# danieldugas/DeepMimic_mujoco

Hardware: AMD Instinct MI355X
Metric: env-steps/sec (whole node), 34-DoF humanoid, 4096 envs, at 1/2/4/8 MI355X (higher is better)
Workload: dtype f32

## Files before the change

### deepmimic_mujoco_amd/csrc/dm_kernels.hip

```cpp
#include "../../include/deepmimic_hip.h"
#include "dm_device.h"
#include "dm_rng.h"
#include "dm_topology.h"

#include <math.h>

#include <type_traits>

#define SYNC()                                              \
  do {                                                      \
    __builtin_amdgcn_fence(__ATOMIC_RELEASE, "wavefront");  \
    __builtin_amdgcn_wave_barrier();                        \
    __builtin_amdgcn_fence(__ATOMIC_ACQUIRE, "wavefront");  \
  } while (0)
#define DMK_ENVS_PER_BLOCK 1
#ifndef DMK_WAVES_PER_SIMD
#define DMK_WAVES_PER_SIMD 2
#endif
#ifdef DM_PROFILE
#define PROF_DECL do { if ((threadIdx.x & 63) == 0) { for (int _i = 0; _i < 16; _i++) g_S.prof[_i] = 0; for (int _i = 0; _i < 4; _i++) g_S.prof_stage[_i] = 0; g_S.prof_t = g_S.prof_t0 = __builtin_amdgcn_s_memtime(); } } while (0)
#define PROF_STAGE(i) do { if ((threadIdx.x & 63) == 0 && (i) < 4) g_S.prof_stage[i] = (unsigned)(__builtin_amdgcn_s_memtime() - g_S.prof_t0); } while (0)
#define PROF(i) do { if ((threadIdx.x & 63) == 0) { unsigned long long _t = __builtin_amdgcn_s_memtime(); g_S.prof[i] += (unsigned)(_t - g_S.prof_t); g_S.prof_t = _t; } } while (0)
#if DM_PROFILE == 2
#define PROF2(i) PROF(i)
// ... 28 lines not shown
namespace {

template <int I, int N>
struct StaticFor {
  template <class F>
  static __device__ __forceinline__ void run(F &&f) {
    if constexpr (I < N) {
      if (f(std::integral_constant<int, I>{})) StaticFor<I + 1, N>::run(f);
    }
  }
};

__device__ __forceinline__ float rl(float v, int lane) {
  return __int_as_float(__builtin_amdgcn_readlane(__float_as_int(v), lane));
}
template <unsigned long long MASK>
__device__ __forceinline__ float lane_sel(float a, float b) {
  float out;
  asm("v_cndmask_b32_e64 %0, %1, %2, %3" : "=v"(out) : "v"(b), "v"(a), "s"(MASK));
  return out;
}
template <unsigned long long MASK>
__device__ __forceinline__ int lane_sel_i(int a, int b) {
  int out;
  asm("v_cndmask_b32_e64 %0, %1, %2, %3" : "=v"(out) : "v"(b), "v"(a), "s"(MASK));
  return out;
}
template <int N>
__device__ __forceinline__ void sgpr_batch(float (&a)[topo::FS_SLOTS]) {
  static_assert(N >= 1 && N <= 8 && topo::FS_SLOTS == 8, "one asm statement per batch size");
  if constexpr (N == 1) asm("" : "+s"(a[0]));
  if constexpr (N == 2) asm("" : "+s"(a[0]), "+s"(a[1]));
  if constexpr (N == 3) asm("" : "+s"(a[0]), "+s"(a[1]), "+s"(a[2]));
  if constexpr (N == 4) asm("" : "+s"(a[0]), "+s"(a[1]), "+s"(a[2]), "+s"(a[3]));
  if constexpr (N == 5) asm("" : "+s"(a[0]), "+s"(a[1]), "+s"(a[2]), "+s"(a[3]), "+s"(a[4]));
  if constexpr (N == 6) asm("" : "+s"(a[0]), "+s"(a[1]), "+s"(a[2]), "+s"(a[3]), "+s"(a[4]), "+s"(a[5]));
  if constexpr (N == 7) asm("" : "+s"(a[0]), "+s"(a[1]), "+s"(a[2]), "+s"(a[3]), "+s"(a[4]), "+s"(a[5]), "+s"(a[6]));
  if constexpr (N == 8) asm("" : "+s"(a[0]), "+s"(a[1]), "+s"(a[2]), "+s"(a[3]), "+s"(a[4]), "+s"(a[5]), "+s"(a[6]), "+s"(a[7]));
}
__device__ __forceinline__ void factor_columns(float (&C)[DMK_NV]) {
  float d[topo::FS_SLOTS], m[topo::FS_SLOTS], rk[DMK_NV], Cs[DMK_NV];
  StaticFor<0, topo::FS_NOPS>::run([&](auto nc) {
    constexpr topo::FactorOp o = topo::FACTOR_SCHED[decltype(nc)::value];
    if constexpr (o.op == topo::FS_DIAG) d[o.slot] = rl(C[o.k], o.k);
    if constexpr (o.op == topo::FS_RCP) rk[o.k] = __builtin_amdgcn_rcpf(d[o.slot]);
    if constexpr (o.op == topo::FS_SCALE) Cs[o.k] = C[o.k] * rk[o.k];
    if constexpr (o.op == topo::FS_BCAST) m[o.slot] = rl(Cs[o.k], o.i);
    if constexpr (o.op == topo::FS_FMA) C[o.i] = fmaf(-m[o.slot], C[o.k], C[o.i]);
    if constexpr (o.op == topo::FS_FENCE) sgpr_batch<o.slot>(m);
    if constexpr (o.op == topo::FS_DFENCE) sgpr_batch<o.slot>(d);
    return true;
  });
}
__device__ __forceinline__ float solve_LT(float x, const float dv, const int negdep, const float *M) {
  StaticFor<0, DMK_NV - 1>::run([&](auto ic) {
    constexpr int i = DMK_NV - 1 - decltype(ic)::value;
    const float xi = rl(x * dv, i);
    const float l = lane_sel<topo::anc_mask(i)>(M[topo::MADR[i] + topo::NANC[i] + negdep], 0.f);
    x = fmaf(-l, xi, x);
    return true;
  });
  return x;
}
__device__ __forceinline__ float solve_L(float x, const float dv, const int mrow, const float *M) {
  StaticFor<0, DMK_NV - 1>::run([&](auto jc) {
    constexpr int j = decltype(jc)::value;
    const float xj = rl(x * dv, j);
    const float l = lane_sel<topo::desc_mask(j)>(M[mrow - topo::NANC[j]], 0.f);
    x = fmaf(-l, xj, x);
    return true;
  });
  return x;
}
template <int I, int K = 0>
__device__ __forceinline__ void load_factor_row(lds_cfloat_p Sp, float (&W)[DMK_MAXANC], float &dinv) {
  static_assert(alignof(EnvLds) >= 16 && offsetof(EnvLds, M) % 4 == 0 && offsetof(EnvLds, dinv) % 4 == 0, "EnvLds layout");
  constexpr int n = topo::NANC[I];
  constexpr int a = (int)(offsetof(EnvLds, M) / 4) + topo::MADR[I] + 1 + K;
  if constexpr (K >= n) {
    dinv = Sp[offsetof(EnvLds, dinv) / 4 + I];
  } else if constexpr (a % 4 == 0 && n - K >= 4) {
    const lds_f4v v = *reinterpret_cast<__attribute__((address_space(3))) const lds_f4v *>(Sp + a);
    W[K] = v.x; W[K + 1] = v.y; W[K + 2] = v.z; W[K + 3] = v.w;
    load_factor_row<I, K + 4>(Sp, W, dinv);
  } else if constexpr (a % 2 == 0 && n - K >= 2) {
    const lds_f2v v = *reinterpret_cast<__attribute__((address_space(3))) const lds_f2v *>(Sp + a);
    W[K] = v.x; W[K + 1] = v.y;
    load_factor_row<I, K + 2>(Sp, W, dinv);
  } else {
    W[K] = Sp[a];
    load_factor_row<I, K + 1>(Sp, W, dinv);
  }
}
template <int CTRL>
__device__ __forceinline__ float dpp_mov(float v) {
  return __int_as_float(__builtin_amdgcn_update_dpp(0, __float_as_int(v), CTRL, 0xF, 0xF, true));
}
__device__ __forceinline__ float wave_sum(float v) {
  v += dpp_mov<0xB1>(v);
  v += dpp_mov<0x4E>(v);
  v += dpp_mov<0x141>(v);
  v += dpp_mov<0x140>(v);
  return (rl(v, 0) + rl(v, 16)) + (rl(v, 32) + rl(v, 48));
}
__device__ __forceinline__ unsigned long long lanemask_lt(int lane) {
  return (lane == 0) ? 0ull : (~0ull >> (64 - lane));
}
__device__ __forceinline__ int prefix_count(bool flag, int lane, int *total) {
  unsigned long long m = __ballot(flag);
  *total = __popcll(m);
  return __popcll(m & lanemask_lt(lane));
}

__device__ __forceinline__ void cross3(float *r, const float *a, const float *b) {
  float x = a[1] * b[2] - a[2] * b[1], y = a[2] * b[0] - a[0] * b[2], z = a[0] * b[1] - a[1] * b[0];
  r[0] = x; r[1] = y; r[2] = z;
}
__device__ __forceinline__ float dot3(const float *a, const float *b) {
  return a[0] * b[0] + a[1] * b[1] + a[2] * b[2];
}
__device__ __forceinline__ void quat_mul(float *r, const float *a, const float *b) {
  float w = a[0] * b[0] - a[1] * b[1] - a[2] * b[2] - a[3] * b[3];
  float x = a[0] * b[1] + a[1] * b[0] + a[2] * b[3] - a[3] * b[2];
  float y = a[0] * b[2] - a[1] * b[3] + a[2] * b[0] + a[3] * b[1];
  float z = a[0] * b[3] + a[1] * b[2] - a[2] * b[1] + a[3] * b[0];
// ... 1867 lines not shown
```

### deepmimic_mujoco_amd/csrc/dm_topology.h

```cpp
#pragma once
namespace topo {
constexpr int NV = 34;
constexpr int NM = 310;
constexpr int PARENT[NV] = {-1, 0, 1, 2, 3, 4, 5, 6, 7, 8, 9, 10, 8, 12, 13, 14, 8, 16, 17, 18, 5, 20, 21, 22, 23, 24, 25, 5, 27, 28, 29, 30, 31, 32};
constexpr int NANC[NV] = {0, 1, 2, 3, 4, 5, 6, 7, 8, 9, 10, 11, 9, 10, 11, 12, 9, 10, 11, 12, 6, 7, 8, 9, 10, 11, 12, 6, 7, 8, 9, 10, 11, 12};
constexpr int MADR[NV] = {0, 1, 3, 6, 10, 15, 21, 28, 36, 45, 55, 66, 78, 88, 99, 111, 124, 134, 145, 157, 170, 177, 185, 194, 204, 215, 227, 240, 247, 255, 264, 274, 285, 297};
constexpr bool is_anc(int j, int i) {
  for (int a = PARENT[i]; a >= 0; a = PARENT[a]) if (a == j) return true;
  return false;
}
constexpr int midx(int i, int j) { return MADR[i] + NANC[i] - NANC[j]; }
constexpr int NB = 14;
constexpr int BPARENT[NB] = {0, 0, 1, 2, 2, 4, 2, 6, 1, 8, 9, 1, 11, 12};
constexpr unsigned long long body_ancself_mask(int c) {
  unsigned long long m = 0;
  for (int b = c; b >= 1; b = BPARENT[b]) m |= 1ull << b;
  return m;
}
constexpr unsigned long long desc_mask(int j) {
  unsigned long long m = 0;
  for (int i = 0; i < NV; i++) if (is_anc(j, i)) m |= 1ull << i;
  return m;
}
constexpr unsigned long long anc_mask(int i) {
// ... 75 lines not shown
  {FS_FMA, 19, 3, 7}, {FS_BCAST, 19, 2, 0}, {FS_BCAST, 19, 1, 1}, {FS_BCAST, 19, 0, 2}, {FS_BCAST, 18, 8, 3}, {FS_BCAST, 18, 7, 4},
  {FS_BCAST, 18, 6, 5}, {FS_BCAST, 18, 5, 6}, {FS_BCAST, 18, 4, 7}, {FS_FENCE, 0, 0, 8}, {FS_FMA, 19, 2, 0}, {FS_FMA, 19, 1, 1},
  {FS_FMA, 19, 0, 2}, {FS_FMA, 18, 8, 3}, {FS_FMA, 18, 7, 4}, {FS_FMA, 18, 6, 5}, {FS_FMA, 18, 5, 6}, {FS_FMA, 18, 4, 7},
  {FS_BCAST, 18, 3, 0}, {FS_BCAST, 18, 2, 1}, {FS_BCAST, 18, 1, 2}, {FS_BCAST, 18, 0, 3}, {FS_BCAST, 17, 8, 4}, {FS_BCAST, 17, 7, 5},
  {FS_BCAST, 17, 6, 6}, {FS_BCAST, 17, 5, 7}, {FS_FENCE, 0, 0, 8}, {FS_FMA, 18, 3, 0}, {FS_FMA, 18, 2, 1}, {FS_FMA, 18, 1, 2},
  {FS_FMA, 18, 0, 3}, {FS_FMA, 17, 8, 4}, {FS_FMA, 17, 7, 5}, {FS_FMA, 17, 6, 6}, {FS_FMA, 17, 5, 7}, {FS_BCAST, 17, 4, 0},
  {FS_BCAST, 17, 3, 1}, {FS_BCAST, 17, 2, 2}, {FS_BCAST, 17, 1, 3}, {FS_BCAST, 17, 0, 4}, {FS_BCAST, 16, 8, 5}, {FS_BCAST, 16, 7, 6},
  {FS_BCAST, 16, 6, 7}, {FS_FENCE, 0, 0, 8}, {FS_FMA, 17, 4, 0}, {FS_FMA, 17, 3, 1}, {FS_FMA, 17, 2, 2}, {FS_FMA, 17, 1, 3},
  {FS_FMA, 17, 0, 4}, {FS_FMA, 16, 8, 5}, {FS_FMA, 16, 7, 6}, {FS_FMA, 16, 6, 7}, {FS_BCAST, 16, 5, 0}, {FS_BCAST, 16, 4, 1},
  {FS_BCAST, 16, 3, 2}, {FS_BCAST, 16, 2, 3}, {FS_BCAST, 16, 1, 4}, {FS_BCAST, 16, 0, 5}, {FS_BCAST, 15, 8, 6}, {FS_BCAST, 15, 7, 7},
  {FS_FENCE, 0, 0, 8}, {FS_FMA, 16, 5, 0}, {FS_FMA, 16, 4, 1}, {FS_FMA, 16, 3, 2}, {FS_FMA, 16, 2, 3}, {FS_FMA, 16, 1, 4},
  {FS_FMA, 16, 0, 5}, {FS_FMA, 15, 8, 6}, {FS_FMA, 15, 7, 7}, {FS_BCAST, 15, 6, 0}, {FS_BCAST, 15, 5, 1}, {FS_BCAST, 15, 4, 2},
  {FS_BCAST, 15, 3, 3}, {FS_BCAST, 15, 2, 4}, {FS_BCAST, 15, 1, 5}, {FS_BCAST, 15, 0, 6}, {FS_BCAST, 14, 8, 7}, {FS_FENCE, 0, 0, 8},
  {FS_FMA, 15, 6, 0}, {FS_FMA, 15, 5, 1}, {FS_FMA, 15, 4, 2}, {FS_FMA, 15, 3, 3}, {FS_FMA, 15, 2, 4}, {FS_FMA, 15, 1, 5},
  {FS_FMA, 15, 0, 6}, {FS_FMA, 14, 8, 7}, {FS_BCAST, 14, 7, 0}, {FS_BCAST, 14, 6, 1}, {FS_BCAST, 14, 5, 2}, {FS_BCAST, 14, 4, 3},
  {FS_BCAST, 14, 3, 4}, {FS_BCAST, 14, 2, 5}, {FS_BCAST, 14, 1, 6}, {FS_BCAST, 14, 0, 7}, {FS_FENCE, 0, 0, 8}, {FS_FMA, 14, 7, 0},
  {FS_FMA, 14, 6, 1}, {FS_FMA, 14, 5, 2}, {FS_FMA, 14, 4, 3}, {FS_FMA, 14, 3, 4}, {FS_FMA, 14, 2, 5}, {FS_FMA, 14, 1, 6},
  {FS_FMA, 14, 0, 7}, {FS_BCAST, 13, 8, 0}, {FS_BCAST, 13, 7, 1}, {FS_BCAST, 13, 6, 2}, {FS_BCAST, 13, 5, 3}, {FS_BCAST, 13, 4, 4},
  {FS_BCAST, 13, 3, 5}, {FS_BCAST, 13, 2, 6}, {FS_BCAST, 13, 1, 7}, {FS_FENCE, 0, 0, 8}, {FS_FMA, 13, 8, 0}, {FS_FMA, 13, 7, 1},
  {FS_FMA, 13, 6, 2}, {FS_FMA, 13, 5, 3}, {FS_FMA, 13, 4, 4}, {FS_FMA, 13, 3, 5}, {FS_FMA, 13, 2, 6}, {FS_FMA, 13, 1, 7},
  {FS_BCAST, 13, 0, 0}, {FS_BCAST, 12, 8, 1}, {FS_BCAST, 12, 7, 2}, {FS_BCAST, 12, 6, 3}, {FS_BCAST, 12, 5, 4}, {FS_BCAST, 12, 4, 5},
  {FS_BCAST, 12, 3, 6}, {FS_BCAST, 12, 2, 7}, {FS_FENCE, 0, 0, 8}, {FS_FMA, 13, 0, 0}, {FS_FMA, 12, 8, 1}, {FS_FMA, 12, 7, 2},
  {FS_FMA, 12, 6, 3}, {FS_FMA, 12, 5, 4}, {FS_FMA, 12, 4, 5}, {FS_FMA, 12, 3, 6}, {FS_FMA, 12, 2, 7}, {FS_BCAST, 12, 1, 0},
  {FS_BCAST, 12, 0, 1}, {FS_BCAST, 11, 8, 2}, {FS_BCAST, 11, 7, 3}, {FS_BCAST, 11, 6, 4}, {FS_BCAST, 11, 5, 5}, {FS_BCAST, 11, 4, 6},
  {FS_BCAST, 11, 3, 7}, {FS_FENCE, 0, 0, 8}, {FS_FMA, 12, 1, 0}, {FS_FMA, 12, 0, 1}, {FS_FMA, 11, 8, 2}, {FS_FMA, 11, 7, 3},
  {FS_FMA, 11, 6, 4}, {FS_FMA, 11, 5, 5}, {FS_FMA, 11, 4, 6}, {FS_FMA, 11, 3, 7}, {FS_BCAST, 11, 2, 0}, {FS_BCAST, 11, 1, 1},
  {FS_BCAST, 11, 0, 2}, {FS_BCAST, 10, 8, 3}, {FS_BCAST, 10, 7, 4}, {FS_BCAST, 10, 6, 5}, {FS_BCAST, 10, 5, 6}, {FS_BCAST, 10, 4, 7},
  {FS_FENCE, 0, 0, 8}, {FS_FMA, 11, 2, 0}, {FS_FMA, 11, 1, 1}, {FS_FMA, 11, 0, 2}, {FS_FMA, 10, 8, 3}, {FS_FMA, 10, 7, 4},
  {FS_FMA, 10, 6, 5}, {FS_FMA, 10, 5, 6}, {FS_FMA, 10, 4, 7}, {FS_BCAST, 10, 3, 0}, {FS_BCAST, 10, 2, 1}, {FS_BCAST, 10, 1, 2},
  {FS_BCAST, 10, 0, 3}, {FS_BCAST, 9, 8, 4}, {FS_BCAST, 9, 7, 5}, {FS_BCAST, 9, 6, 6}, {FS_BCAST, 9, 5, 7}, {FS_FENCE, 0, 0, 8},
  {FS_FMA, 10, 3, 0}, {FS_FMA, 10, 2, 1}, {FS_FMA, 10, 1, 2}, {FS_FMA, 10, 0, 3}, {FS_FMA, 9, 8, 4}, {FS_FMA, 9, 7, 5},
  {FS_FMA, 9, 6, 6}, {FS_FMA, 9, 5, 7}, {FS_BCAST, 9, 4, 0}, {FS_BCAST, 9, 3, 1}, {FS_BCAST, 9, 2, 2}, {FS_BCAST, 9, 1, 3},
  {FS_BCAST, 9, 0, 4}, {FS_FENCE, 0, 0, 5}, {FS_FMA, 9, 4, 0}, {FS_FMA, 9, 3, 1}, {FS_FMA, 9, 2, 2}, {FS_FMA, 9, 1, 3},
  {FS_FMA, 9, 0, 4}, {FS_DIAG, 8, 8, 0}, {FS_DFENCE, 0, 0, 1}, {FS_RCP, 8, 8, 0}, {FS_SCALE, 8, 8, 0}, {FS_BCAST, 8, 7, 0},
  {FS_BCAST, 8, 6, 1}, {FS_BCAST, 8, 5, 2}, {FS_BCAST, 8, 4, 3}, {FS_BCAST, 8, 3, 4}, {FS_BCAST, 8, 2, 5}, {FS_BCAST, 8, 1, 6},
  {FS_BCAST, 8, 0, 7}, {FS_FENCE, 0, 0, 8}, {FS_FMA, 8, 7, 0}, {FS_FMA, 8, 6, 1}, {FS_FMA, 8, 5, 2}, {FS_FMA, 8, 4, 3},
  {FS_FMA, 8, 3, 4}, {FS_FMA, 8, 2, 5}, {FS_FMA, 8, 1, 6}, {FS_FMA, 8, 0, 7}, {FS_DIAG, 7, 7, 0}, {FS_DFENCE, 0, 0, 1},
  {FS_RCP, 7, 7, 0}, {FS_SCALE, 7, 7, 0}, {FS_BCAST, 7, 6, 0}, {FS_BCAST, 7, 5, 1}, {FS_BCAST, 7, 4, 2}, {FS_BCAST, 7, 3, 3},
  {FS_BCAST, 7, 2, 4}, {FS_BCAST, 7, 1, 5}, {FS_BCAST, 7, 0, 6}, {FS_FENCE, 0, 0, 7}, {FS_FMA, 7, 6, 0}, {FS_FMA, 7, 5, 1},
  {FS_FMA, 7, 4, 2}, {FS_FMA, 7, 3, 3}, {FS_FMA, 7, 2, 4}, {FS_FMA, 7, 1, 5}, {FS_FMA, 7, 0, 6}, {FS_DIAG, 6, 6, 0},
  {FS_DFENCE, 0, 0, 1}, {FS_RCP, 6, 6, 0}, {FS_SCALE, 6, 6, 0}, {FS_BCAST, 6, 5, 0}, {FS_BCAST, 6, 4, 1}, {FS_BCAST, 6, 3, 2},
  {FS_BCAST, 6, 2, 3}, {FS_BCAST, 6, 1, 4}, {FS_BCAST, 6, 0, 5}, {FS_FENCE, 0, 0, 6}, {FS_FMA, 6, 5, 0}, {FS_FMA, 6, 4, 1},
  {FS_FMA, 6, 3, 2}, {FS_FMA, 6, 2, 3}, {FS_FMA, 6, 1, 4}, {FS_FMA, 6, 0, 5}, {FS_DIAG, 5, 5, 0}, {FS_DFENCE, 0, 0, 1},
  {FS_RCP, 5, 5, 0}, {FS_SCALE, 5, 5, 0}, {FS_BCAST, 5, 4, 0}, {FS_BCAST, 5, 3, 1}, {FS_BCAST, 5, 2, 2}, {FS_BCAST, 5, 1, 3},
  {FS_BCAST, 5, 0, 4}, {FS_FENCE, 0, 0, 5}, {FS_FMA, 5, 4, 0}, {FS_FMA, 5, 3, 1}, {FS_FMA, 5, 2, 2}, {FS_FMA, 5, 1, 3},
  {FS_FMA, 5, 0, 4}, {FS_DIAG, 4, 4, 0}, {FS_DFENCE, 0, 0, 1}, {FS_RCP, 4, 4, 0}, {FS_SCALE, 4, 4, 0}, {FS_BCAST, 4, 3, 0},
  {FS_BCAST, 4, 2, 1}, {FS_BCAST, 4, 1, 2}, {FS_BCAST, 4, 0, 3}, {FS_FENCE, 0, 0, 4}, {FS_FMA, 4, 3, 0}, {FS_FMA, 4, 2, 1},
  {FS_FMA, 4, 1, 2}, {FS_FMA, 4, 0, 3}, {FS_DIAG, 3, 3, 0}, {FS_DFENCE, 0, 0, 1}, {FS_RCP, 3, 3, 0}, {FS_SCALE, 3, 3, 0},
  {FS_BCAST, 3, 2, 0}, {FS_BCAST, 3, 1, 1}, {FS_BCAST, 3, 0, 2}, {FS_FENCE, 0, 0, 3}, {FS_FMA, 3, 2, 0}, {FS_FMA, 3, 1, 1},
  {FS_FMA, 3, 0, 2}, {FS_DIAG, 2, 2, 0}, {FS_DFENCE, 0, 0, 1}, {FS_RCP, 2, 2, 0}, {FS_SCALE, 2, 2, 0}, {FS_BCAST, 2, 1, 0},
  {FS_BCAST, 2, 0, 1}, {FS_FENCE, 0, 0, 2}, {FS_FMA, 2, 1, 0}, {FS_FMA, 2, 0, 1}, {FS_DIAG, 1, 1, 0}, {FS_DFENCE, 0, 0, 1},
  {FS_RCP, 1, 1, 0}, {FS_SCALE, 1, 1, 0}, {FS_BCAST, 1, 0, 0}, {FS_FENCE, 0, 0, 1}, {FS_FMA, 1, 0, 0},
};
}
```

### deepmimic_mujoco_amd/gen_topology.py

```python
import os

from .model import NV, NBODY, load_model

OUT = os.path.join(os.path.dirname(os.path.abspath(__file__)), "csrc", "dm_topology.h")

FS_DIAG, FS_RCP, FS_SCALE, FS_BCAST, FS_FMA, FS_FENCE, FS_DFENCE = range(7)
FS_SLOTS = 8


def factor_schedule(parent, slots=FS_SLOTS):
    nv = len(parent)
    kids = [[c for c in range(nv) if parent[c] == k] for k in range(nv)]
    anc = []
    for k in range(nv):
        a, l = parent[k], []
        while a >= 0:
            l.append(a)
            a = parent[a]
        anc.append(l)
    trunk = [k for k in range(nv) if any(len(kids[j]) > 1 for j in range(nv) if j == k or k in anc[j])]
    limbs = []
    for k in reversed(range(nv)):
        if k not in trunk and not kids[k]:
            limb = [k]
            while parent[limb[-1]] not in trunk and parent[limb[-1]] >= 0:
                limb.append(parent[limb[-1]])
            limbs.append(limb)
    ops = []

    def heads(ks, stages):
        for op in stages:
            for s, k in enumerate(ks):
                ops.append((op, k, k, s))
            if op == FS_DIAG and ks:
                ops.append((FS_DFENCE, 0, 0, len(ks)))

    def batches(pairs):
        return [pairs[b:b + slots] for b in range(0, len(pairs), slots)]

    def updates(batch):
        for s, (k, i) in enumerate(batch):
            ops.append((FS_BCAST, k, i, s))
        ops.append((FS_FENCE, 0, 0, len(batch)))
        for s, (k, i) in enumerate(batch):
            ops.append((FS_FMA, k, i, s))

    first = limbs[0] if limbs and all(min(limbs[0]) > max(l) for l in limbs[1:]) else None
    assert len(limbs) <= slots
    rounds = [[l[r] for l in limbs if len(l) > r] for r in range(max((len(l) for l in limbs), default=0))]
    for r, piv in enumerate(rounds):
        nxt = rounds[r + 1] if r + 1 < len(rounds) else []
        if r == 0:
            heads(piv, (FS_DIAG, FS_RCP, FS_SCALE))
        own = {k: [i for i in anc[k] if i not in trunk or k in (first or ())] for k in piv}
        todo = batches([(k, own[k][0]) for k in piv if own[k]] + [(k, i) for k in piv for i in own[k][1:]])
        for n, batch in enumerate(todo):
            updates(batch)
            if n == 0:
                heads(nxt, (FS_DIAG,))
            if n == min(1, len(todo) - 1):
                heads(nxt, (FS_RCP, FS_SCALE))
    later = sorted((k for l in limbs if l is not first for k in l), reverse=True)
    for batch in batches([(k, i) for k in later for i in anc[k] if i in trunk]):
        updates(batch)
    for k in sorted(trunk, reverse=True):
        if k >= 1:
            heads([k], (FS_DIAG, FS_RCP, FS_SCALE))
            for batch in batches([(k, i) for i in anc[k]]):
                updates(batch)
    check_factor_schedule(parent, ops)
    return ops


def check_factor_schedule(parent, ops):
    nv = len(parent)
    anc = {k: [] for k in range(nv)}
    for k in range(nv):
        a = parent[k]
        while a >= 0:
            anc[k].append(a)
            a = parent[a]
    pairs = [(k, i) for k in range(nv) for i in anc[k]]
    fmas = [(k, i) for op, k, i, s in ops if op == FS_FMA]
    assert sorted(fmas) == sorted(pairs), "the updates are not a permutation of the (dof, ancestor) pairs"
    for op in (FS_DIAG, FS_RCP, FS_SCALE):
        assert sorted(k for o, k, i, s in ops if o == op) == list(range(1, nv)), "every dof 1.. has one pivot"
    last = {i: nv for i in range(nv)}
    left = {i: sum(1 for p in pairs if p[1] == i) for i in range(nv)}
    slot, dslot, have = {}, {}, {k: set() for k in range(nv)}
    for n, (op, k, i, s) in enumerate(ops):
        if op == FS_DIAG:
            assert left[k] == 0, "op %d: pivot %d before the last update into C[%d]" % (n, k, k)
            dslot[s] = (k, False)
        elif op == FS_RCP:
            assert dslot.get(s) == (k, True), "op %d: rcp of dof %d reads slot %d, which does not hold its fenced diagonal" % (n, k, s)
            have[k].add(FS_RCP)
        elif op == FS_SCALE:
            assert FS_RCP in have[k], "op %d: scale of dof %d before its rcp" % (n, k)
            have[k].add(FS_SCALE)
        elif op == FS_BCAST:
            assert FS_SCALE in have[k] and i in anc[k], "op %d: broadcast (%d, %d)" % (n, k, i)
            slot[s] = (k, i, False)
        elif op == FS_FENCE:
            for t in range(s):
                slot[t] = slot[t][:2] + (True,)
        elif op == FS_DFENCE:
            for t in range(s):
                dslot[t] = (dslot[t][0], True)
        elif op == FS_FMA:
            assert slot.get(s) == (k, i, True), "op %d: update (%d, %d) reads slot %d, which does not hold its fenced multiplier" % (n, k, i, s)
            assert k < last[i], "op %d: update (%d, %d) after the update of dof %d into C[%d]" % (n, k, i, last[i], i)
            last[i] = k
            left[i] -= 1
    return True


def render(model):
    parent = [int(x) for x in model.dof_parent]
    nanc = []
    for k in range(NV):
        n, a = 0, parent[k]
        while a >= 0:
            n += 1
            a = parent[a]
        nanc.append(n)
    madr = [int(x) for x in model.dof_Madr]
    bparent = [int(x) for x in model.body_parent]
    lines = [
        "// GENERATED by deepmimic_mujoco_amd/gen_topology.py from deepmimic_humanoid3d.xml — do not edit.",
        "// Dof tree of the model (reference: mjModel.dof_parentid / dof_Madr of the asset loaded at",
        "// src/deepmimic_env.py:301).  Sparse inertia layout: row i = M(i,i), M(i,parent), M(i,grandparent), ...",
        "#pragma once",
        "namespace topo {",
        "constexpr int NV = %d;" % NV,
        "constexpr int NM = %d;" % (madr[-1] + nanc[-1] + 1),
        "constexpr int PARENT[NV] = {%s};" % ", ".join(map(str, parent)),
        "constexpr int NANC[NV] = {%s};" % ", ".join(map(str, nanc)),
        "constexpr int MADR[NV] = {%s};" % ", ".join(map(str, madr)),
        "constexpr bool is_anc(int j, int i) {  // j is a strict ancestor of i",
        "  for (int a = PARENT[i]; a >= 0; a = PARENT[a]) if (a == j) return true;",
        "  return false;",
        "}",
        "constexpr int midx(int i, int j) { return MADR[i] + NANC[i] - NANC[j]; }  // j ancestor-or-self of i",
        "constexpr int NB = %d;" % NBODY,
        "constexpr int BPARENT[NB] = {%s};  // body tree (body 0 = world)" % ", ".join(map(str, bparent)),
        "constexpr unsigned long long body_ancself_mask(int c) {  // bit b: body b (>= 1) is c or an ancestor of c",
        "  unsigned long long m = 0;",
        "  for (int b = c; b >= 1; b = BPARENT[b]) m |= 1ull << b;",
        "  return m;",
        "}",
        "constexpr unsigned long long desc_mask(int j) {  // bit i: dof i is a strict descendant of j",
        "  unsigned long long m = 0;",
        "  for (int i = 0; i < NV; i++) if (is_anc(j, i)) m |= 1ull << i;",
        "  return m;",
        "}",
        "constexpr unsigned long long anc_mask(int i) {  // bit j: dof j is a strict ancestor of i (= the lanes that own M[i][j])",
        "  unsigned long long m = 0;",
        "  for (int a = PARENT[i]; a >= 0; a = PARENT[a]) m |= 1ull << a;",
        "  return m;",
        "}",
    ]
    sched = factor_schedule(parent)
    lines += [
        "// Emission order of the L^T D L elimination in fwd_smooth: a topological order of its dependency DAG in which the",
        "// limbs run side by side and the broadcasts of a batch precede their FMAs (gen_topology.factor_schedule).",
        "enum { FS_DIAG, FS_RCP, FS_SCALE, FS_BCAST, FS_FMA, FS_FENCE, FS_DFENCE };",
        "struct FactorOp { unsigned char op, k, i, slot; };",
        "constexpr int FS_SLOTS = %d;" % FS_SLOTS,
        "constexpr int FS_NOPS = %d;" % len(sched),
        "constexpr FactorOp FACTOR_SCHED[FS_NOPS] = {",
    ]
    names = ("FS_DIAG", "FS_RCP", "FS_SCALE", "FS_BCAST", "FS_FMA", "FS_FENCE", "FS_DFENCE")
    for b in range(0, len(sched), 6):
        lines.append("  " + " ".join("{%s, %d, %d, %d}," % (names[op], k, i, s) for op, k, i, s in sched[b:b + 6]))
    lines += [
        "};",
        "}  // namespace topo",
        "",
    ]
    return "\n".join(lines)


OUT_G1 = os.path.join(os.path.dirname(os.path.abspath(__file__)), "csrc", "dm_g1_topology.h")


def render_g1(g):
    parent = [int(x) for x in g.dof_parent]
    madr = [int(x) for x in g.dof_Madr]
    nanc = []
    for k in range(g.nv):
        n, a = 0, parent[k]
        while a >= 0:
            n, a = n + 1, parent[a]
        nanc.append(n)
    return "\n".join([
        "// GENERATED by deepmimic_mujoco_amd/gen_topology.py from deepmimic_unitree_g1.xml — do not edit.",
        "// Dof tree of the Unitree G1 model: with it known at compile time the constraint rows are solved against the sparse",
        "// factor in registers (static indices).  dmg1_create() rejects a model whose dof tree differs.",
        "#pragma once",
        "namespace g1topo {",
        "constexpr int NV = %d;" % g.nv,
        "constexpr int PARENT[NV] = {%s};" % ", ".join(map(str, parent)),
        "constexpr int NANC[NV] = {%s};" % ", ".join(map(str, nanc)),
        "constexpr int MADR[NV] = {%s};" % ", ".join(map(str, madr)),
        "}  // namespace g1topo",
        "",
    ])


def _write(path, txt):
    old = open(path).read() if os.path.exists(path) else None
    if old != txt:
        with open(path, "w") as f:
            f.write(txt)


def main():
    _write(OUT, render(load_model()))
    from . import mjcf
    from .model import ASSET_DIR
    _write(OUT_G1, render_g1(mjcf.compile_mjcf_general(os.path.join(ASSET_DIR, "deepmimic_unitree_g1.xml"))))
    return OUT


if __name__ == "__main__":
    print(main())
```

Before: 14.61 million.

## Schedule triangular solves by tree level with prefetched factor loads

Replaces the serial 33-step forward solve_L with a generated schedule that processes all dofs of the same depth level in one round. The round's scalars are broadcast together behind a single SGPR fence, and factor entries are loaded from memory ahead of use into a small register array. A matching limb-parallel schedule for solve_LT is added with a trunk copy and merge, but it sits behind a macro that defaults to off. The goal is a shorter serial dependency chain and hidden load latency in the per-env solve, at the cost of more live registers.

```diff
diff --git a/deepmimic_mujoco_amd/csrc/dm_kernels.hip b/deepmimic_mujoco_amd/csrc/dm_kernels.hip
--- a/deepmimic_mujoco_amd/csrc/dm_kernels.hip
+++ b/deepmimic_mujoco_amd/csrc/dm_kernels.hip
@@ -104,7 +104,34 @@
     return true;
   });
 }
+template <bool LT>
+__device__ __forceinline__ float solve_sched(float x, const float dv, const int base, const float *M) {
+  constexpr const topo::SolveOp *tab = LT ? topo::SOLVE_LT_SCHED : topo::SOLVE_L_SCHED;
+  float s[topo::FS_SLOTS], ld[topo::SS_LSLOTS], xs = 0.f, xt = x;
+  StaticFor<0, (LT ? topo::SS_LT_NOPS : topo::SS_L_NOPS)>::run([&](auto nc) {
+    constexpr topo::SolveOp o = tab[decltype(nc)::value];
+    if constexpr (o.op == topo::SS_LOAD) ld[o.lslot] = LT ? M[topo::MADR[o.k] + topo::NANC[o.k] + base] : M[base - o.k];
+    if constexpr (o.op == topo::SS_SCALE) xs = x * dv;
+    if constexpr (o.op == topo::SS_BCAST) s[o.slot] = rl(xs, o.k);
+    if constexpr (o.op == topo::SS_FENCE) sgpr_batch<o.slot>(s);
+    if constexpr (o.op == topo::SS_FMA) {
+      constexpr unsigned long long mask = topo::solve_mask(o.kind, o.k);
+      static_assert((mask == 0) == (o.lslot == topo::SS_NOLOAD), "an entry is loaded for every non-empty mask");
+      float l = 0.f;
+      if constexpr (mask != 0) l = lane_sel<mask>(ld[o.lslot], 0.f);
+      if constexpr (o.kind == topo::SM_TRUNK) xt = fmaf(-l, s[o.slot], xt);
+      else x = fmaf(-l, s[o.slot], x);
+    }
+    if constexpr (o.op == topo::SS_MERGE) x = lane_sel<topo::TRUNK_MASK>(xt, x);
+    return true;
+  });
+  return x;
+}
+#ifndef DMK_SOLVE_LT_SCHED
+#define DMK_SOLVE_LT_SCHED 0
+#endif
 __device__ __forceinline__ float solve_LT(float x, const float dv, const int negdep, const float *M) {
+  if constexpr (DMK_SOLVE_LT_SCHED) return solve_sched<true>(x, dv, negdep, M);
   StaticFor<0, DMK_NV - 1>::run([&](auto ic) {
     constexpr int i = DMK_NV - 1 - decltype(ic)::value;
     const float xi = rl(x * dv, i);
@@ -115,14 +142,7 @@
   return x;
 }
 __device__ __forceinline__ float solve_L(float x, const float dv, const int mrow, const float *M) {
-  StaticFor<0, DMK_NV - 1>::run([&](auto jc) {
-    constexpr int j = decltype(jc)::value;
-    const float xj = rl(x * dv, j);
-    const float l = lane_sel<topo::desc_mask(j)>(M[mrow - topo::NANC[j]], 0.f);
-    x = fmaf(-l, xj, x);
-    return true;
-  });
-  return x;
+  return solve_sched<false>(x, dv, mrow, M);
 }
 template <int I, int K = 0>
 __device__ __forceinline__ void load_factor_row(lds_cfloat_p Sp, float (&W)[DMK_MAXANC], float &dinv) {
diff --git a/deepmimic_mujoco_amd/csrc/dm_topology.h b/deepmimic_mujoco_amd/csrc/dm_topology.h
--- a/deepmimic_mujoco_amd/csrc/dm_topology.h
+++ b/deepmimic_mujoco_amd/csrc/dm_topology.h
@@ -151,4 +151,81 @@
   {FS_BCAST, 2, 0, 1}, {FS_FENCE, 0, 0, 2}, {FS_FMA, 2, 1, 0}, {FS_FMA, 2, 0, 1}, {FS_DIAG, 1, 1, 0}, {FS_DFENCE, 0, 0, 1},
   {FS_RCP, 1, 1, 0}, {FS_SCALE, 1, 1, 0}, {FS_BCAST, 1, 0, 0}, {FS_FENCE, 0, 0, 1}, {FS_FMA, 1, 0, 0},
 };
-}
+enum { SS_LOAD, SS_SCALE, SS_BCAST, SS_FENCE, SS_FMA, SS_MERGE };
+enum { SM_DESC, SM_LIMB, SM_TRUNK, SM_ANC };
+struct SolveOp { unsigned char op, k, slot, lslot, kind; };
+constexpr int SS_NOLOAD = 255;
+constexpr int SS_LSLOTS = 16;
+constexpr unsigned long long TRUNK_MASK = 0x1ffull;
+constexpr unsigned long long solve_mask(int kind, int k) {
+  return kind == SM_DESC ? desc_mask(k) : kind == SM_LIMB ? anc_mask(k) & ~TRUNK_MASK : kind == SM_TRUNK ? anc_mask(k) & TRUNK_MASK : anc_mask(k);
+}
+constexpr int SS_L_NOPS = 104;
+constexpr SolveOp SOLVE_L_SCHED[SS_L_NOPS] = {
+  {SS_LOAD, 0, 0, 0, SM_DESC}, {SS_LOAD, 1, 0, 1, SM_DESC}, {SS_LOAD, 2, 0, 2, SM_DESC}, {SS_LOAD, 3, 0, 3, SM_DESC}, {SS_SCALE, 0, 0, 255, SM_DESC},
+  {SS_BCAST, 0, 0, 255, SM_DESC}, {SS_FENCE, 0, 1, 255, SM_DESC}, {SS_FMA, 0, 0, 0, SM_DESC}, {SS_SCALE, 0, 0, 255, SM_DESC}, {SS_BCAST, 1, 0, 255, SM_DESC},
+  {SS_FENCE, 0, 1, 255, SM_DESC}, {SS_FMA, 1, 0, 1, SM_DESC}, {SS_LOAD, 4, 0, 0, SM_DESC}, {SS_LOAD, 5, 0, 1, SM_DESC}, {SS_SCALE, 0, 0, 255, SM_DESC},
+  {SS_BCAST, 2, 0, 255, SM_DESC}, {SS_FENCE, 0, 1, 255, SM_DESC}, {SS_FMA, 2, 0, 2, SM_DESC}, {SS_SCALE, 0, 0, 255, SM_DESC}, {SS_BCAST, 3, 0, 255, SM_DESC},
+  {SS_FENCE, 0, 1, 255, SM_DESC}, {SS_FMA, 3, 0, 3, SM_DESC}, {SS_LOAD, 6, 0, 2, SM_DESC}, {SS_LOAD, 7, 0, 3, SM_DESC}, {SS_SCALE, 0, 0, 255, SM_DESC},
+  {SS_BCAST, 4, 0, 255, SM_DESC}, {SS_FENCE, 0, 1, 255, SM_DESC}, {SS_FMA, 4, 0, 0, SM_DESC}, {SS_SCALE, 0, 0, 255, SM_DESC}, {SS_BCAST, 5, 0, 255, SM_DESC},
+  {SS_FENCE, 0, 1, 255, SM_DESC}, {SS_FMA, 5, 0, 1, SM_DESC}, {SS_LOAD, 8, 0, 0, SM_DESC}, {SS_LOAD, 9, 0, 1, SM_DESC}, {SS_SCALE, 0, 0, 255, SM_DESC},
+  {SS_BCAST, 6, 0, 255, SM_DESC}, {SS_BCAST, 20, 1, 255, SM_DESC}, {SS_BCAST, 27, 2, 255, SM_DESC}, {SS_FENCE, 0, 3, 255, SM_DESC}, {SS_FMA, 6, 0, 2, SM_DESC},
+  {SS_FMA, 20, 1, 2, SM_DESC}, {SS_FMA, 27, 2, 2, SM_DESC}, {SS_SCALE, 0, 0, 255, SM_DESC}, {SS_BCAST, 7, 0, 255, SM_DESC}, {SS_BCAST, 21, 1, 255, SM_DESC},
+  {SS_BCAST, 28, 2, 255, SM_DESC}, {SS_FENCE, 0, 3, 255, SM_DESC}, {SS_FMA, 7, 0, 3, SM_DESC}, {SS_FMA, 21, 1, 3, SM_DESC}, {SS_FMA, 28, 2, 3, SM_DESC},
+  {SS_LOAD, 10, 0, 2, SM_DESC}, {SS_LOAD, 11, 0, 3, SM_DESC}, {SS_SCALE, 0, 0, 255, SM_DESC}, {SS_BCAST, 8, 0, 255, SM_DESC}, {SS_BCAST, 22, 1, 255, SM_DESC},
+  {SS_BCAST, 29, 2, 255, SM_DESC}, {SS_FENCE, 0, 3, 255, SM_DESC}, {SS_FMA, 8, 0, 0, SM_DESC}, {SS_FMA, 22, 1, 0, SM_DESC}, {SS_FMA, 29, 2, 0, SM_DESC},
+  {SS_SCALE, 0, 0, 255, SM_DESC}, {SS_BCAST, 9, 0, 255, SM_DESC}, {SS_BCAST, 12, 1, 255, SM_DESC}, {SS_BCAST, 16, 2, 255, SM_DESC}, {SS_BCAST, 23, 3, 255, SM_DESC},
+  {SS_BCAST, 30, 4, 255, SM_DESC}, {SS_FENCE, 0, 5, 255, SM_DESC}, {SS_FMA, 9, 0, 1, SM_DESC}, {SS_FMA, 12, 1, 1, SM_DESC}, {SS_FMA, 16, 2, 1, SM_DESC},
+  {SS_FMA, 23, 3, 1, SM_DESC}, {SS_FMA, 30, 4, 1, SM_DESC}, {SS_SCALE, 0, 0, 255, SM_DESC}, {SS_BCAST, 10, 0, 255, SM_DESC}, {SS_BCAST, 13, 1, 255, SM_DESC},
+  {SS_BCAST, 17, 2, 255, SM_DESC}, {SS_BCAST, 24, 3, 255, SM_DESC}, {SS_BCAST, 31, 4, 255, SM_DESC}, {SS_FENCE, 0, 5, 255, SM_DESC}, {SS_FMA, 10, 0, 2, SM_DESC},
+  {SS_FMA, 13, 1, 2, SM_DESC}, {SS_FMA, 17, 2, 2, SM_DESC}, {SS_FMA, 24, 3, 2, SM_DESC}, {SS_FMA, 31, 4, 2, SM_DESC}, {SS_SCALE, 0, 0, 255, SM_DESC},
+  {SS_BCAST, 11, 0, 255, SM_DESC}, {SS_BCAST, 14, 1, 255, SM_DESC}, {SS_BCAST, 18, 2, 255, SM_DESC}, {SS_BCAST, 25, 3, 255, SM_DESC}, {SS_BCAST, 32, 4, 255, SM_DESC},
+  {SS_FENCE, 0, 5, 255, SM_DESC}, {SS_FMA, 11, 0, 255, SM_DESC}, {SS_FMA, 14, 1, 3, SM_DESC}, {SS_FMA, 18, 2, 3, SM_DESC}, {SS_FMA, 25, 3, 3, SM_DESC},
+  {SS_FMA, 32, 4, 3, SM_DESC}, {SS_SCALE, 0, 0, 255, SM_DESC}, {SS_BCAST, 15, 0, 255, SM_DESC}, {SS_BCAST, 19, 1, 255, SM_DESC}, {SS_BCAST, 26, 2, 255, SM_DESC},
+  {SS_FENCE, 0, 3, 255, SM_DESC}, {SS_FMA, 15, 0, 255, SM_DESC}, {SS_FMA, 19, 1, 255, SM_DESC}, {SS_FMA, 26, 2, 255, SM_DESC},
+};
+constexpr int SS_LT_NOPS = 205;
+constexpr SolveOp SOLVE_LT_SCHED[SS_LT_NOPS] = {
+  {SS_LOAD, 11, 0, 0, SM_DESC}, {SS_LOAD, 15, 0, 1, SM_DESC}, {SS_LOAD, 19, 0, 2, SM_DESC}, {SS_LOAD, 26, 0, 3, SM_DESC}, {SS_LOAD, 33, 0, 4, SM_DESC},
+  {SS_LOAD, 10, 0, 5, SM_DESC}, {SS_LOAD, 14, 0, 6, SM_DESC}, {SS_LOAD, 18, 0, 7, SM_DESC}, {SS_LOAD, 25, 0, 8, SM_DESC}, {SS_LOAD, 32, 0, 9, SM_DESC},
+  {SS_SCALE, 0, 0, 255, SM_DESC}, {SS_BCAST, 33, 0, 255, SM_DESC}, {SS_BCAST, 26, 1, 255, SM_DESC}, {SS_BCAST, 19, 2, 255, SM_DESC}, {SS_BCAST, 15, 3, 255, SM_DESC},
+  {SS_BCAST, 11, 4, 255, SM_DESC}, {SS_FENCE, 0, 5, 255, SM_DESC}, {SS_FMA, 33, 0, 4, SM_LIMB}, {SS_FMA, 26, 1, 3, SM_LIMB}, {SS_FMA, 19, 2, 2, SM_LIMB},
+  {SS_FMA, 15, 3, 1, SM_LIMB}, {SS_FMA, 11, 4, 0, SM_LIMB}, {SS_LOAD, 13, 0, 0, SM_DESC}, {SS_LOAD, 17, 0, 1, SM_DESC}, {SS_LOAD, 24, 0, 2, SM_DESC},
+  {SS_LOAD, 31, 0, 3, SM_DESC}, {SS_SCALE, 0, 0, 255, SM_DESC}, {SS_BCAST, 32, 0, 255, SM_DESC}, {SS_BCAST, 25, 1, 255, SM_DESC}, {SS_BCAST, 18, 2, 255, SM_DESC},
+  {SS_BCAST, 14, 3, 255, SM_DESC}, {SS_BCAST, 10, 4, 255, SM_DESC}, {SS_FENCE, 0, 5, 255, SM_DESC}, {SS_FMA, 32, 0, 9, SM_LIMB}, {SS_FMA, 25, 1, 8, SM_LIMB},
+  {SS_FMA, 18, 2, 7, SM_LIMB}, {SS_FMA, 14, 3, 6, SM_LIMB}, {SS_FMA, 10, 4, 5, SM_LIMB}, {SS_LOAD, 23, 0, 4, SM_DESC}, {SS_LOAD, 30, 0, 5, SM_DESC},
+  {SS_SCALE, 0, 0, 255, SM_DESC}, {SS_BCAST, 31, 0, 255, SM_DESC}, {SS_BCAST, 24, 1, 255, SM_DESC}, {SS_BCAST, 17, 2, 255, SM_DESC}, {SS_BCAST, 13, 3, 255, SM_DESC},
+  {SS_BCAST, 9, 4, 255, SM_DESC}, {SS_FENCE, 0, 5, 255, SM_DESC}, {SS_FMA, 31, 0, 3, SM_LIMB}, {SS_FMA, 24, 1, 2, SM_LIMB}, {SS_FMA, 17, 2, 1, SM_LIMB},
+  {SS_FMA, 13, 3, 0, SM_LIMB}, {SS_FMA, 9, 4, 255, SM_LIMB}, {SS_LOAD, 22, 0, 0, SM_DESC}, {SS_LOAD, 29, 0, 1, SM_DESC}, {SS_SCALE, 0, 0, 255, SM_DESC},
+  {SS_BCAST, 30, 0, 255, SM_DESC}, {SS_BCAST, 23, 1, 255, SM_DESC}, {SS_BCAST, 16, 2, 255, SM_DESC}, {SS_BCAST, 12, 3, 255, SM_DESC}, {SS_FENCE, 0, 4, 255, SM_DESC},
+  {SS_FMA, 30, 0, 5, SM_LIMB}, {SS_FMA, 23, 1, 4, SM_LIMB}, {SS_FMA, 16, 2, 255, SM_LIMB}, {SS_FMA, 12, 3, 255, SM_LIMB}, {SS_LOAD, 21, 0, 2, SM_DESC},
+  {SS_LOAD, 28, 0, 3, SM_DESC}, {SS_SCALE, 0, 0, 255, SM_DESC}, {SS_BCAST, 29, 0, 255, SM_DESC}, {SS_BCAST, 22, 1, 255, SM_DESC}, {SS_FENCE, 0, 2, 255, SM_DESC},
+  {SS_FMA, 29, 0, 1, SM_LIMB}, {SS_FMA, 22, 1, 0, SM_LIMB}, {SS_SCALE, 0, 0, 255, SM_DESC}, {SS_BCAST, 28, 0, 255, SM_DESC}, {SS_BCAST, 21, 1, 255, SM_DESC},
+  {SS_FENCE, 0, 2, 255, SM_DESC}, {SS_FMA, 28, 0, 3, SM_LIMB}, {SS_FMA, 21, 1, 2, SM_LIMB}, {SS_LOAD, 26, 0, 0, SM_DESC}, {SS_LOAD, 27, 0, 1, SM_DESC},
+  {SS_LOAD, 28, 0, 2, SM_DESC}, {SS_LOAD, 29, 0, 3, SM_DESC}, {SS_LOAD, 30, 0, 4, SM_DESC}, {SS_LOAD, 31, 0, 5, SM_DESC}, {SS_LOAD, 32, 0, 6, SM_DESC},
+  {SS_LOAD, 33, 0, 7, SM_DESC}, {SS_SCALE, 0, 0, 255, SM_DESC}, {SS_BCAST, 27, 0, 255, SM_DESC}, {SS_BCAST, 20, 1, 255, SM_DESC}, {SS_FENCE, 0, 2, 255, SM_DESC},
+  {SS_FMA, 27, 0, 255, SM_LIMB}, {SS_FMA, 20, 1, 255, SM_LIMB}, {SS_LOAD, 18, 0, 8, SM_DESC}, {SS_LOAD, 19, 0, 9, SM_DESC}, {SS_LOAD, 20, 0, 10, SM_DESC},
+  {SS_LOAD, 21, 0, 11, SM_DESC}, {SS_LOAD, 22, 0, 12, SM_DESC}, {SS_LOAD, 23, 0, 13, SM_DESC}, {SS_LOAD, 24, 0, 14, SM_DESC}, {SS_LOAD, 25, 0, 15, SM_DESC},
+  {SS_SCALE, 0, 0, 255, SM_DESC}, {SS_BCAST, 33, 0, 255, SM_DESC}, {SS_BCAST, 32, 1, 255, SM_DESC}, {SS_BCAST, 31, 2, 255, SM_DESC}, {SS_BCAST, 30, 3, 255, SM_DESC},
+  {SS_BCAST, 29, 4, 255, SM_DESC}, {SS_BCAST, 28, 5, 255, SM_DESC}, {SS_BCAST, 27, 6, 255, SM_DESC}, {SS_BCAST, 26, 7, 255, SM_DESC}, {SS_FENCE, 0, 8, 255, SM_DESC},
+  {SS_FMA, 33, 0, 7, SM_TRUNK}, {SS_FMA, 32, 1, 6, SM_TRUNK}, {SS_FMA, 31, 2, 5, SM_TRUNK}, {SS_FMA, 30, 3, 4, SM_TRUNK}, {SS_FMA, 29, 4, 3, SM_TRUNK},
+  {SS_FMA, 28, 5, 2, SM_TRUNK}, {SS_FMA, 27, 6, 1, SM_TRUNK}, {SS_FMA, 26, 7, 0, SM_TRUNK}, {SS_LOAD, 10, 0, 0, SM_DESC}, {SS_LOAD, 11, 0, 1, SM_DESC},
+  {SS_LOAD, 12, 0, 2, SM_DESC}, {SS_LOAD, 13, 0, 3, SM_DESC}, {SS_LOAD, 14, 0, 4, SM_DESC}, {SS_LOAD, 15, 0, 5, SM_DESC}, {SS_LOAD, 16, 0, 6, SM_DESC},
+  {SS_LOAD, 17, 0, 7, SM_DESC}, {SS_BCAST, 25, 0, 255, SM_DESC}, {SS_BCAST, 24, 1, 255, SM_DESC}, {SS_BCAST, 23, 2, 255, SM_DESC}, {SS_BCAST, 22, 3, 255, SM_DESC},
+  {SS_BCAST, 21, 4, 255, SM_DESC}, {SS_BCAST, 20, 5, 255, SM_DESC}, {SS_BCAST, 19, 6, 255, SM_DESC}, {SS_BCAST, 18, 7, 255, SM_DESC}, {SS_FENCE, 0, 8, 255, SM_DESC},
+  {SS_FMA, 25, 0, 15, SM_TRUNK}, {SS_FMA, 24, 1, 14, SM_TRUNK}, {SS_FMA, 23, 2, 13, SM_TRUNK}, {SS_FMA, 22, 3, 12, SM_TRUNK}, {SS_FMA, 21, 4, 11, SM_TRUNK},
+  {SS_FMA, 20, 5, 10, SM_TRUNK}, {SS_FMA, 19, 6, 9, SM_TRUNK}, {SS_FMA, 18, 7, 8, SM_TRUNK}, {SS_LOAD, 9, 0, 8, SM_DESC}, {SS_BCAST, 17, 0, 255, SM_DESC},
+  {SS_BCAST, 16, 1, 255, SM_DESC}, {SS_BCAST, 15, 2, 255, SM_DESC}, {SS_BCAST, 14, 3, 255, SM_DESC}, {SS_BCAST, 13, 4, 255, SM_DESC}, {SS_BCAST, 12, 5, 255, SM_DESC},
+  {SS_BCAST, 11, 6, 255, SM_DESC}, {SS_BCAST, 10, 7, 255, SM_DESC}, {SS_FENCE, 0, 8, 255, SM_DESC}, {SS_FMA, 17, 0, 7, SM_TRUNK}, {SS_FMA, 16, 1, 6, SM_TRUNK},
+  {SS_FMA, 15, 2, 5, SM_TRUNK}, {SS_FMA, 14, 3, 4, SM_TRUNK}, {SS_FMA, 13, 4, 3, SM_TRUNK}, {SS_FMA, 12, 5, 2, SM_TRUNK}, {SS_FMA, 11, 6, 1, SM_TRUNK},
+  {SS_FMA, 10, 7, 0, SM_TRUNK}, {SS_LOAD, 8, 0, 0, SM_DESC}, {SS_LOAD, 7, 0, 1, SM_DESC}, {SS_BCAST, 9, 0, 255, SM_DESC}, {SS_FENCE, 0, 1, 255, SM_DESC},
+  {SS_FMA, 9, 0, 8, SM_TRUNK}, {SS_MERGE, 0, 0, 255, SM_DESC}, {SS_LOAD, 6, 0, 2, SM_DESC}, {SS_LOAD, 5, 0, 3, SM_DESC}, {SS_SCALE, 0, 0, 255, SM_DESC},
+  {SS_BCAST, 8, 0, 255, SM_DESC}, {SS_FENCE, 0, 1, 255, SM_DESC}, {SS_FMA, 8, 0, 0, SM_ANC}, {SS_SCALE, 0, 0, 255, SM_DESC}, {SS_BCAST, 7, 0, 255, SM_DESC},
+  {SS_FENCE, 0, 1, 255, SM_DESC}, {SS_FMA, 7, 0, 1, SM_ANC}, {SS_LOAD, 4, 0, 0, SM_DESC}, {SS_LOAD, 3, 0, 1, SM_DESC}, {SS_SCALE, 0, 0, 255, SM_DESC},
+  {SS_BCAST, 6, 0, 255, SM_DESC}, {SS_FENCE, 0, 1, 255, SM_DESC}, {SS_FMA, 6, 0, 2, SM_ANC}, {SS_SCALE, 0, 0, 255, SM_DESC}, {SS_BCAST, 5, 0, 255, SM_DESC},
+  {SS_FENCE, 0, 1, 255, SM_DESC}, {SS_FMA, 5, 0, 3, SM_ANC}, {SS_LOAD, 2, 0, 2, SM_DESC}, {SS_LOAD, 1, 0, 3, SM_DESC}, {SS_SCALE, 0, 0, 255, SM_DESC},
+  {SS_BCAST, 4, 0, 255, SM_DESC}, {SS_FENCE, 0, 1, 255, SM_DESC}, {SS_FMA, 4, 0, 0, SM_ANC}, {SS_SCALE, 0, 0, 255, SM_DESC}, {SS_BCAST, 3, 0, 255, SM_DESC},
+  {SS_FENCE, 0, 1, 255, SM_DESC}, {SS_FMA, 3, 0, 1, SM_ANC}, {SS_SCALE, 0, 0, 255, SM_DESC}, {SS_BCAST, 2, 0, 255, SM_DESC}, {SS_FENCE, 0, 1, 255, SM_DESC},
+  {SS_FMA, 2, 0, 2, SM_ANC}, {SS_SCALE, 0, 0, 255, SM_DESC}, {SS_BCAST, 1, 0, 255, SM_DESC}, {SS_FENCE, 0, 1, 255, SM_DESC}, {SS_FMA, 1, 0, 3, SM_ANC},
+};
+}
diff --git a/deepmimic_mujoco_amd/gen_topology.py b/deepmimic_mujoco_amd/gen_topology.py
--- a/deepmimic_mujoco_amd/gen_topology.py
+++ b/deepmimic_mujoco_amd/gen_topology.py
@@ -10,22 +10,7 @@
 
 def factor_schedule(parent, slots=FS_SLOTS):
     nv = len(parent)
-    kids = [[c for c in range(nv) if parent[c] == k] for k in range(nv)]
-    anc = []
-    for k in range(nv):
-        a, l = parent[k], []
-        while a >= 0:
-            l.append(a)
-            a = parent[a]
-        anc.append(l)
-    trunk = [k for k in range(nv) if any(len(kids[j]) > 1 for j in range(nv) if j == k or k in anc[j])]
-    limbs = []
-    for k in reversed(range(nv)):
-        if k not in trunk and not kids[k]:
-            limb = [k]
-            while parent[limb[-1]] not in trunk and parent[limb[-1]] >= 0:
-                limb.append(parent[limb[-1]])
-            limbs.append(limb)
+    anc, trunk, limbs = _tree(parent)
     ops = []
 
     def heads(ks, stages):
@@ -115,6 +100,155 @@
     return True
 
 
+SS_LOAD, SS_SCALE, SS_BCAST, SS_FENCE, SS_FMA, SS_MERGE = range(6)
+SM_DESC, SM_LIMB, SM_TRUNK, SM_ANC = range(4)
+SS_NOLOAD = 255
+SS_AHEAD = 2
+SS_BATCH_AHEAD = 1
+
+
+def _tree(parent):
+    nv = len(parent)
+    kids = [[c for c in range(nv) if parent[c] == k] for k in range(nv)]
+    anc = []
+    for k in range(nv):
+        a, l = parent[k], []
+        while a >= 0:
+            l.append(a)
+            a = parent[a]
+        anc.append(l)
+    trunk = [k for k in range(nv) if any(len(kids[j]) > 1 for j in range(nv) if j == k or k in anc[j])]
+    limbs = []
+    for k in reversed(range(nv)):
+        if k not in trunk and not kids[k]:
+            limb = [k]
+            while parent[limb[-1]] not in trunk and parent[limb[-1]] >= 0:
+                limb.append(parent[limb[-1]])
+            limbs.append(limb)
+    return anc, trunk, limbs
+
+
+def solve_mask(parent, kind, k):
+    anc, trunk, _ = _tree(parent)
+    if kind == SM_DESC:
+        return [i for i in range(len(parent)) if k in anc[i]]
+    return [j for j in anc[k] if kind == SM_ANC or (j in trunk) == (kind == SM_TRUNK)]
+
+
+def _emit_rounds(rounds, slots):
+    ops, held, free, top = [], {}, [], 0
+    for r, (_, _, body) in enumerate(rounds):
+        for at, keys, _ in rounds:
+            if at == r:
+                for key in keys:
+                    if free:
+                        held[key] = free.pop(0)
+                    else:
+                        held[key], top = top, top + 1
+                    ops.append((SS_LOAD, key[1], 0, held[key], 0))
+        last = {key: n for n, (op, k, s, key, kind) in enumerate(body) if key is not None}
+        for n, (op, k, s, key, kind) in enumerate(body):
+            ops.append((op, k, s, SS_NOLOAD if key is None else held[key], kind))
+            if key is not None and last[key] == n:
+                free.append(held.pop(key))
+                free.sort()
+    assert not held and all(0 <= o[2] <= slots for o in ops)
+    return ops
+
+
+def _serial_request(first, r):
+    return max(first - 1, 0, first + 2 * ((r - first) // 2) - SS_AHEAD)
+
+
+def solve_schedule(parent, slots=FS_SLOTS):
+    nv = len(parent)
+    anc, trunk, limbs = _tree(parent)
+    depth = [len(a) for a in anc]
+    desc = [[i for i in range(nv) if k in anc[i]] for k in range(nv)]
+
+    def round_of(ks, kind, masks, key_of, scale=True):
+        body = [(SS_SCALE, 0, 0, None, 0)] if scale else []
+        body += [(SS_BCAST, k, s, None, 0) for s, k in enumerate(ks)] + [(SS_FENCE, 0, len(ks), None, 0)]
+        body += [(SS_FMA, k, s, key_of(k) if masks[k] else None, kind) for s, k in enumerate(ks)]
+        return sorted({key_of(k) for k in ks if masks[k]}), body
+
+    levels = [[j for j in range(nv - 1) if depth[j] == d] for d in range(max(depth) + 1)]
+    levels = [l for l in levels if l]
+    assert all(len(l) <= slots for l in levels)
+    rounds = []
+    for r, ks in enumerate(levels):
+        keys, body = round_of(ks, SM_DESC, desc, lambda k: ("d", depth[k]))
+        rounds.append((_serial_request(0, r), keys, body))
+    ops_l = _emit_rounds(rounds, slots)
+
+    rounds = []
+    nlimb = max((len(l) for l in limbs), default=0)
+    own = {k: [j for j in anc[k] if j not in trunk] for k in range(nv)}
+    tr = {k: [j for j in anc[k] if j in trunk] for k in range(nv)}
+    for r in range(nlimb):
+        keys, body = round_of([l[r] for l in limbs if len(l) > r], SM_LIMB, own, lambda k: ("a", k))
+        rounds.append((max(0, r - SS_BATCH_AHEAD), keys, body))
+    later = sorted((k for l in limbs for k in l), reverse=True)
+    for b in range(0, len(later), slots):
+        keys, body = round_of(later[b:b + slots], SM_TRUNK, tr, lambda k: ("b", k), scale=(b == 0))
+        rounds.append((len(rounds) - SS_BATCH_AHEAD, keys, body))
+    rounds[-1][2].append((SS_MERGE, 0, 0, None, 0))
+    first_c = len(rounds)
+    for k in sorted(trunk, reverse=True):
+        if k >= 1:
+            keys, body = round_of([k], SM_ANC, anc, lambda k: ("c", k))
+            rounds.append((_serial_request(first_c, len(rounds)), keys, body))
+    ops_lt = _emit_rounds(rounds, slots)
+    check_solve_schedule(parent, ops_l, ops_lt)
+    return ops_l, ops_lt
+
+
+def check_solve_schedule(parent, ops_l, ops_lt):
+    nv = len(parent)
+    anc, trunk, _ = _tree(parent)
+    depth = [len(a) for a in anc]
+    for lt, ops in ((False, ops_l), (True, ops_lt)):
+        srcs = list(range(nv - 1, 0, -1)) if lt else list(range(nv - 1))
+        want = {i: [k for k in srcs if (i in anc[k] if lt else k in anc[i])] for i in range(nv)}
+        real = {"x": {i: [] for i in range(nv)}, "xt": {i: [] for i in range(nv)}}
+        zero = {"x": {i: [] for i in range(nv)}, "xt": {i: [] for i in range(nv)}}
+        xs, s, ld = None, {}, {}
+        for n, (op, k, slot, lslot, kind) in enumerate(ops):
+            if op == SS_LOAD:
+                ld[lslot] = k
+            elif op == SS_SCALE:
+                xs = {i: list(real["x"][i]) for i in range(nv)}
+            elif op == SS_BCAST:
+                assert xs is not None and xs[k] == want[k], "op %d: broadcast of dof %d before the last update into its lane" % (n, k)
+                s[slot] = (k, False)
+            elif op == SS_FENCE:
+                for t in range(slot):
+                    s[t] = (s[t][0], True)
+            elif op == SS_FMA:
+                assert s.get(slot) == (k, True), "op %d: FMA of dof %d reads slot %d, which does not hold its fenced scalar" % (n, k, slot)
+                assert kind == SM_DESC if not lt else kind in (SM_LIMB, SM_TRUNK, SM_ANC), "op %d: mask kind %d" % (n, kind)
+                lanes = solve_mask(parent, kind, k)
+                if lanes:
+                    assert ld.get(lslot) == (k if lt else depth[k]), "op %d: FMA of dof %d reads load slot %d, which does not hold its entry" % (n, k, lslot)
+                else:
+                    assert lslot == SS_NOLOAD, "op %d: an entry for an empty mask" % n
+                reg = "xt" if kind == SM_TRUNK else "x"
+                for i in range(nv):
+                    (real if i in lanes else zero)[reg][i].append(k)
+                    if i in lanes:
+                        assert real[reg][i] == want[i][:len(real[reg][i])], "op %d: update of dof %d into lane %d out of order" % (n, k, i)
+            elif op == SS_MERGE:
+                for i in trunk:
+                    assert not real["x"][i], "op %d: x's trunk lane %d was updated before the merge" % (n, i)
+                    real["x"][i], zero["x"][i] = real["xt"][i], zero["xt"][i]
+            else:
+                raise AssertionError("op %d: unknown op %d" % (n, op))
+        for i in range(nv):
+            assert real["x"][i] == want[i], "lane %d ends with the updates %s" % (i, real["x"][i])
+            assert sorted(real["x"][i] + zero["x"][i]) == sorted(srcs), "lane %d does not see every step once" % i
+    return True
+
+
 def render(model):
     parent = [int(x) for x in model.dof_parent]
     nanc = []
@@ -173,8 +307,30 @@
     names = ("FS_DIAG", "FS_RCP", "FS_SCALE", "FS_BCAST", "FS_FMA", "FS_FENCE", "FS_DFENCE")
     for b in range(0, len(sched), 6):
         lines.append("  " + " ".join("{%s, %d, %d, %d}," % (names[op], k, i, s) for op, k, i, s in sched[b:b + 6]))
+    lines.append("};")
+    ops_l, ops_lt = solve_schedule(parent)
+    _, trunk, _ = _tree(parent)
     lines += [
-        "};",
+        "// Emission order of the triangular solves solve_L (by depth level) and solve_LT (limbs side by side, their updates into the",
+        "// trunk on the copy xt, the trunk serially), factor entries requested ahead of their round (gen_topology.solve_schedule).",
+        "enum { SS_LOAD, SS_SCALE, SS_BCAST, SS_FENCE, SS_FMA, SS_MERGE };",
+        "enum { SM_DESC, SM_LIMB, SM_TRUNK, SM_ANC };",
+        "struct SolveOp { unsigned char op, k, slot, lslot, kind; };",
+        "constexpr int SS_NOLOAD = %d;" % SS_NOLOAD,
+        "constexpr int SS_LSLOTS = %d;" % (1 + max(o[3] for o in ops_l + ops_lt if o[3] != SS_NOLOAD)),
+        "constexpr unsigned long long TRUNK_MASK = 0x%xull;" % sum(1 << k for k in trunk),
+        "constexpr unsigned long long solve_mask(int kind, int k) {",
+        "  return kind == SM_DESC ? desc_mask(k) : kind == SM_LIMB ? anc_mask(k) & ~TRUNK_MASK : kind == SM_TRUNK ? anc_mask(k) & TRUNK_MASK : anc_mask(k);",
+        "}",
+    ]
+    snames = ("SS_LOAD", "SS_SCALE", "SS_BCAST", "SS_FENCE", "SS_FMA", "SS_MERGE")
+    knames = ("SM_DESC", "SM_LIMB", "SM_TRUNK", "SM_ANC")
+    for tag, ops in (("L", ops_l), ("LT", ops_lt)):
+        lines += ["constexpr int SS_%s_NOPS = %d;" % (tag, len(ops)), "constexpr SolveOp SOLVE_%s_SCHED[SS_%s_NOPS] = {" % (tag, tag)]
+        for b in range(0, len(ops), 5):
+            lines.append("  " + " ".join("{%s, %d, %d, %d, %s}," % (snames[op], k, s, ls, knames[kind]) for op, k, s, ls, kind in ops[b:b + 5]))
+        lines.append("};")
+    lines += [
         "}  // namespace topo",
         "",
     ]
```

Measured after the change: 14.79 million, median of 6. 1.2% higher.
